# RalphAS/PeriodicSchurDecompositions.jl

Measured on NVIDIA B200. Metric: pschur!/sec batched (p=8,N=32); large-N FP64 % peak in large_n, higher is better.
Workload: dtype f64

## Files before the change

### periodicschurdecompositions.jl_b200/csrc/psd_capi.cu

```cuda
#include <algorithm>
#include <atomic>
#include <chrono>
#include <cstdio>
#include <cstdlib>
#include <cstring>
#include <mutex>
#include <string>
#include <thread>
#include <vector>

#include "../../include/psd_b200.h"
#include "psd_real_kernel.cuh"
#include "psd_checkpsd.cuh"
#include "psd_real_hess32.cuh"
#include "psd_cplx_qz.cuh"
#include "psd_rowhess.cuh"
#include "psd_dgemm.cuh"
#include "psd_large_hess.cuh"
#include "psd_ms.h"
#include "psd_rng.cuh"

namespace {

thread_local std::string g_err;
// ... 15 lines not shown
#define PSD_CUDA(call)                                                                     \
  do {                                                                                     \
    cudaError_t e__ = (call);                                                              \
    if (e__ != cudaSuccess)                                                                \
      return fail(PSD_ERR_CUDA, std::string(#call) + ": " + cudaGetErrorString(e__));      \
  } while (0)

constexpr int kSlotsPerDevice = 3;

struct Slot {
  cudaStream_t stream = nullptr;
  double* dA = nullptr;
  double* dZ = nullptr;
  double* dEig = nullptr;
  int32_t* dInfo = nullptr;
  size_t capA = 0, capZ = 0, capEig = 0, capInfo = 0;
  double* hA = nullptr;
  double* hZ = nullptr;
  double* hEig = nullptr;
  int32_t* hInfo = nullptr;
  size_t hcapA = 0, hcapZ = 0, hcapEig = 0, hcapInfo = 0;
  unsigned long long* dCounter = nullptr;
  double* dScratch = nullptr;
  size_t capScratch = 0;
  double* dPacked = nullptr;
  size_t capPacked = 0;
  double* dPk[8] = {nullptr};
  size_t capPk[8] = {0};
  unsigned long long* dPhaseCtr = nullptr;
  void* dX[3] = {nullptr, nullptr, nullptr};
  size_t capX[3] = {0, 0, 0};
  void* hX[3] = {nullptr, nullptr, nullptr};
  size_t hcapX[3] = {0, 0, 0};
  unsigned char* dS = nullptr;
  size_t capS = 0;
  psd::ms::Workspace* ms = nullptr;
  int32_t* dIters = nullptr;
  int32_t* hIters = nullptr;
  size_t capIters = 0, hcapIters = 0;
  int32_t* curIters = nullptr;
  double* curTau = nullptr;
  long long* dProf = nullptr;
};

struct Device {
  int ordinal = 0;
  int sm_count = 0;
  Slot slots[kSlotsPerDevice];
  Slot user;
  cudaEvent_t userDone = nullptr;
};

}

struct KernelTimer {
  cudaEvent_t e0, e1;
  int kind;
  int ordinal;
};

struct psd_handle_s {
  std::vector<Device> devs;
  std::mutex mu;
  int64_t stats[8] = {0};
  bool profiling = false;
  std::vector<KernelTimer> timers;
  double gemm_flops = 0.0;
  double extra_launches = 0.0;
  psd::ms::Result ms_last;
  int32_t* iters_host = nullptr;
  std::mutex tmu;
};

namespace {

template <class T>
int ensure_dev(T*& ptr, size_t& cap, size_t bytes) {
  if (bytes <= cap) return PSD_OK;
  if (ptr) cudaFree(ptr);
  ptr = nullptr;
  cap = 0;
  PSD_CUDA(cudaMalloc((void**)&ptr, bytes));
  cap = bytes;
  return PSD_OK;
}
template <class T>
int ensure_pinned(T*& ptr, size_t& cap, size_t bytes) {
  if (bytes <= cap) return PSD_OK;
  if (ptr) cudaFreeHost(ptr);
  ptr = nullptr;
  cap = 0;
  PSD_CUDA(cudaHostAlloc((void**)&ptr, bytes, cudaHostAllocDefault));
  cap = bytes;
  return PSD_OK;
}

bool is_pinned(const void* p) {
  if (!p) return true;
  cudaPointerAttributes at;
  cudaError_t e = cudaPointerGetAttributes(&at, p);
  if (e != cudaSuccess) {
    cudaGetLastError();
    return false;
  }
  return at.type == cudaMemoryTypeHost || at.type == cudaMemoryTypeManaged;
}

struct ScopedKernelTimer {
  psd_handle_s* h;
  cudaStream_t st;
  KernelTimer t;
  bool on;
  ScopedKernelTimer(psd_handle_s* h_, const Device& dev, cudaStream_t st_, int kind) : h(h_), st(st_) {
    on = h->profiling;
    if (!on) return;
    t.kind = kind;
    t.ordinal = dev.ordinal;
    cudaEventCreate(&t.e0);
    cudaEventCreate(&t.e1);
    cudaEventRecord(t.e0, st);
  }
  ~ScopedKernelTimer() {
    if (!on) return;
    cudaEventRecord(t.e1, st);
    std::lock_guard<std::mutex> lk(h->tmu);
    h->timers.push_back(t);
  }
};

struct RealLaunchPlan {
  int use_smem = 0;
  int ldh = 0;
  int threads = 64;
  size_t smem_bytes = 0;
  int grid = 1;
  bool scratch = false;
};

int plan_real(const Device& dev, int n, int p, long long batch, bool wantZ, RealLaunchPlan& pl) {
  const long long small = psd::rp_small_doubles(n, p);
  const int ldh = (n % 2 == 0) ? n + 1 : n;
  const long long mats = (long long)p * ldh * n * (wantZ ? 2 : 1);
  const size_t need_smem = (size_t)(small + mats) * sizeof(double);
  cudaFuncAttributes fa;
  PSD_CUDA(cudaFuncGetAttributes(&fa, psd::rpschur_kernel));
  int optin = 0;
  PSD_CUDA(cudaDeviceGetAttribute(&optin, cudaDevAttrMaxSharedMemoryPerBlockOptin, dev.ordinal));
  const size_t max_dyn = (size_t)optin - fa.sharedSizeBytes;
  if (need_smem <= max_dyn) {
    pl.use_smem = 1;
    pl.ldh = ldh;
    pl.smem_bytes = need_smem;
    pl.scratch = false;
  } else {
    pl.use_smem = 0;
    pl.ldh = n;
    if ((size_t)small * sizeof(double) <= 96 * 1024) {
      pl.smem_bytes = (size_t)small * sizeof(double);
      pl.scratch = false;
    } else {
      pl.smem_bytes = 0;
      pl.scratch = true;
    }
  }
  int want = n * (wantZ ? 3 : 2);
  int threads = ((want + 31) / 32) * 32;
  threads = std::max(32, std::min(threads, 256));
  pl.threads = threads;
  PSD_CUDA(cudaFuncSetAttribute(psd::rpschur_kernel, cudaFuncAttributeMaxDynamicSharedMemorySize,
                                (int)max_dyn));
  int occ = 0;
  PSD_CUDA(cudaOccupancyMaxActiveBlocksPerMultiprocessor(&occ, psd::rpschur_kernel, threads,
                                                         pl.smem_bytes));
  if (occ < 1) return fail(PSD_ERR_UNSUPPORTED, "kernel does not fit on an SM");
  long long g = (long long)occ * dev.sm_count;
  pl.grid = (int)std::max(1LL, std::min(g, batch));
  return PSD_OK;
}

struct RealCall {
  int n, p, left, wantT, wantZ, maxitfac, reduce_only, skip_reduce;
  int z_preset = 0;
};

constexpr int kLargeN = 192;

constexpr long long kEigChunk = 65536;

int launch_real_eig32(psd_handle_s* h, Device& dev, Slot& aux, cudaStream_t stream, const RealCall& rc,
                      long long batch, double* dA, double* dEig, int32_t* dInfo) {
  const int n = rc.n, p = rc.p;
  const size_t nn = (size_t)n * n;
  const size_t psize = (size_t)psd::pk_problem_size(n, p);
  long long chunk_max = kEigChunk;
  if (const char* ev = dbg_env("PSD_EIG_CHUNK")) chunk_max = std::max(1LL, atoll(ev));
  const long long chunk = std::min(batch, chunk_max);
  int e = ensure_dev(aux.dPacked, aux.capPacked, (size_t)chunk * psd::pk_problem_stride(n, p) * sizeof(double));
  if (e) return e;
  if (!aux.dCounter) PSD_CUDA(cudaMalloc((void**)&aux.dCounter, 2 * sizeof(unsigned long long)));
  if (!aux.dPhaseCtr) PSD_CUDA(cudaMalloc((void**)&aux.dPhaseCtr, 16 * sizeof(unsigned long long)));
  int optin = 0;
  PSD_CUDA(cudaDeviceGetAttribute(&optin, cudaDevAttrMaxSharedMemoryPerBlockOptin, dev.ordinal));
  struct Phase {
    int n, stop, wpb, grid;
    size_t smem;
    void (*kern)(psd::EigParams);
  };
  std::vector<Phase> phases;
  {
    std::vector<int> orders{n};
    if (n >= 24 && !dbg_env("PSD_NO_PHASES"))
      for (int k = 1; k <= 5; k++) orders.push_back(n - k * (n / 8));
    bool special = (n == 32 && p == 8 && !dbg_env("PSD_NO_SPECIAL"));
    if (const char* ev = dbg_env("PSD_PHASES")) {
      orders.assign(1, n);
      for (const char* c = ev; *c;) {
        int v = atoi(c);
        if (v > 1 && v < orders.back()) orders.push_back(v);
        while (*c && *c != ',') c++;
        if (*c == ',') c++;
      }
    }
    for (size_t k = 0; k < orders.size(); k++) {
      Phase ph;
      ph.n = orders[k];
      ph.stop = (k + 1 < orders.size()) ? orders[k + 1] : 0;
      ph.kern = psd::rpqr_eig32_kernel_t<0, 0>;
      if (special && k == 0) ph.kern = psd::rpqr_eig32_kernel_t<32, 8>;
      int wmax = 8;
      if (k > 0) {
        const char* lr = dbg_env("PSD_LOWREG");
        const int mode = lr ? atoi(lr) : 168;
        if (mode == 168) { ph.kern = psd::rpqr_eig32_kernel_r168; wmax = 3; }
        if (mode == 128) { ph.kern = psd::rpqr_eig32_kernel_r128; wmax = 4; }
      }
      cudaFuncAttributes fa;
      PSD_CUDA(cudaFuncGetAttributes(&fa, ph.kern));
      const size_t max_dyn = (size_t)optin - fa.sharedSizeBytes;
      const size_t pbytes = (size_t)psd::pk_problem_size(ph.n, p) * sizeof(double);
      PSD_CUDA(cudaFuncSetAttribute(ph.kern, cudaFuncAttributeMaxDynamicSharedMemorySize, (int)max_dyn));
      PSD_CUDA(cudaFuncSetAttribute(ph.kern, cudaFuncAttributePreferredSharedMemoryCarveout,
                                    (int)cudaSharedmemCarveoutMaxShared));
      int best_w = 0, best_total = 0;
      for (int w = 1; w <= wmax; w++) {
        if ((size_t)w * pbytes > max_dyn) break;
        int occ = 0;
        PSD_CUDA(cudaOccupancyMaxActiveBlocksPerMultiprocessor(&occ, ph.kern, w * 32, (size_t)w * pbytes));
        if (dbg_env("PSD_GEN_PROF")) fprintf(stderr, "[psd eig32 occ] order %d w %d -> %d CTAs/SM\n", ph.n, w, occ);
        if (occ * w > best_total || (occ * w == best_total && w > best_w)) {
          best_total = occ * w;
          best_w = w;
        }
      }
      if (best_w < 1) return fail(PSD_ERR_UNSUPPORTED, "packed problem does not fit in shared memory");
      if (const char* ev = dbg_env("PSD_PHASE_WPB")) {
        const int w = atoi(ev);
        if (k > 0 && w >= 1 && (size_t)w * pbytes <= max_dyn) {
          best_w = w;
          best_total = w * 4;
        }
      }
      ph.wpb = best_w;
      ph.smem = (size_t)best_w * pbytes;
      ph.grid = (best_total / best_w) * dev.sm_count;
      if (dbg_env("PSD_GEN_PROF"))
        fprintf(stderr, "[psd eig32 phase %zu] order %d stop %d: %d warps/CTA x %d CTAs/SM, %zu B smem/CTA, %d regs\n", k,
                ph.n, ph.stop, best_w, best_total / best_w, ph.smem, fa.numRegs);
      phases.push_back(ph);
    }
    if (phases.size() > 9) return fail(PSD_ERR_BAD_ARG, "too many phases");
    for (size_t k = 1; k < phases.size(); k++)
      if ((e = ensure_dev(aux.dPk[k - 1], aux.capPk[k - 1],
                          (size_t)chunk * psd::pk_problem_stride(phases[k].n, p) * sizeof(double))))
        return e;
  }
  for (long long off = 0; off < batch; off += chunk) {
    const long long nb = std::min(chunk, batch - off);
    PSD_CUDA(cudaMemsetAsync(aux.dCounter, 0, 2 * sizeof(unsigned long long), stream));
    if (rc.skip_reduce) {
      RealLaunchPlan pl;
      e = plan_real(dev, n, p, nb, false, pl);
      if (e) return e;
      if (!pl.use_smem) return fail(PSD_ERR_UNSUPPORTED, "eig32 path expects shared-memory staging");
      psd::RpschurParams P;
      P.n = n; P.p = p; P.batch = nb;
      P.left = rc.left; P.wantT = 0; P.wantZ = 0; P.maxitfac = 30;
      P.A = dA + (size_t)off * p * nn; P.Z = nullptr; P.eig = nullptr; P.info = nullptr; P.iters = nullptr;
      P.use_smem = pl.use_smem; P.ldh = pl.ldh;
      P.reduce_only = 1; P.skip_reduce = rc.skip_reduce; P.z_preset = 0;
      P.counter = aux.dCounter;
      P.scratch = nullptr; P.scratch_stride = 0;
      P.packed_out = aux.dPacked;
      P.tau = nullptr;
      ScopedKernelTimer tm(h, dev, stream, 0);
      psd::rpschur_kernel<<<pl.grid, pl.threads, pl.smem_bytes, stream>>>(P);
      PSD_CUDA(cudaGetLastError());
    } else {
      psd::Hess32Params R;
      R.n = n; R.p = p; R.batch = nb; R.left = rc.left;
      R.ld = (n % 2 == 0) ? n + 1 : n;
      R.A = dA + (size_t)off * p * nn;
      R.packed_out = aux.dPacked;
      R.counter = aux.dCounter;
      const bool pair = p >= 2 && !dbg_env("PSD_NO_HESS_PAIR");
      const bool special = n == 32 && p == 8 && !dbg_env("PSD_NO_SPECIAL");
      void (*hk)(psd::Hess32Params) =
          pair ? (special ? psd::rphess_pair32_kernel_t<32, 8> : psd::rphess_pair32_kernel_t<0, 0>)
               : (special ? psd::rphess_warp32_kernel_t<32, 8> : psd::rphess_warp32_kernel_t<0, 0>);
      const int wpp = pair ? 2 : 1;
      cudaFuncAttributes fh;
      PSD_CUDA(cudaFuncGetAttributes(&fh, hk));
      const size_t max_dyn1 = (size_t)optin - fh.sharedSizeBytes;
      const size_t per1 = (size_t)p * R.ld * n * sizeof(double);
      int wpb1 = (int)std::min<size_t>(8, max_dyn1 / per1);
      if (wpb1 < 1) return fail(PSD_ERR_UNSUPPORTED, "problem does not fit in shared memory");
      const size_t smem1 = (size_t)wpb1 * per1;
      PSD_CUDA(cudaFuncSetAttribute(hk, cudaFuncAttributeMaxDynamicSharedMemorySize,
                                    (int)max_dyn1));
      int occ1 = 0;
      PSD_CUDA(cudaOccupancyMaxActiveBlocksPerMultiprocessor(&occ1, hk, wpb1 * wpp * 32, smem1));
      if (occ1 < 1) return fail(PSD_ERR_UNSUPPORTED, "reduction kernel does not fit on an SM");
      const long long ctas1 = (nb + wpb1 - 1) / wpb1;
      const int grid1 = (int)std::max(1LL, std::min((long long)occ1 * dev.sm_count, ctas1));
      {
        ScopedKernelTimer tm(h, dev, stream, 0);
        hk<<<grid1, wpb1 * wpp * 32, smem1, stream>>>(R);
      }
      PSD_CUDA(cudaGetLastError());
    }
    PSD_CUDA(cudaMemsetAsync(aux.dPhaseCtr, 0, 16 * sizeof(unsigned long long), stream));
    {
      ScopedKernelTimer tm(h, dev, stream, 1);
      for (size_t k = 0; k < phases.size(); k++) {
        const Phase& ph = phases[k];
        psd::EigParams Q;
        Q.n = ph.n; Q.p = p; Q.batch = nb; Q.maxitfac = rc.maxitfac > 0 ? rc.maxitfac : 30;
        Q.packed = (k == 0) ? aux.dPacked : aux.dPk[k - 1];
        Q.packed_next = (k + 1 < phases.size()) ? aux.dPk[k] : nullptr;
        Q.n_full = n; Q.stop = ph.stop; Q.first_phase = (k == 0) ? 1 : 0;
        Q.eig = dEig + (size_t)off * 2 * n;
        Q.info = dInfo + off;
        Q.iters = aux.curIters ? aux.curIters + off : nullptr;
        Q.counter = aux.dPhaseCtr + k;
        Q.force_safe = dbg_env("PSD_EIG32_SAFE") ? 1 : 0;
        const long long ctas = (nb + ph.wpb - 1) / ph.wpb;
        const int grid2 = (int)std::max(1LL, std::min((long long)ph.grid, ctas));
        ph.kern<<<grid2, ph.wpb * 32, ph.smem, stream>>>(Q);
      }
    }
    PSD_CUDA(cudaGetLastError());
    {
      std::lock_guard<std::mutex> lk(h->tmu);
      h->extra_launches += (double)(phases.size() - 1);
    }
    __atomic_fetch_add(&h->stats[0], (int64_t)2, __ATOMIC_RELAXED);
  }
  __atomic_fetch_add(&h->stats[1], (int64_t)batch, __ATOMIC_RELAXED);
  return PSD_OK;
}


int launch_real_large(psd_handle_s* h, Device& dev, Slot& aux, cudaStream_t stream, const RealCall& rc,
                      long long batch, double* dA, double* dZ, double* dEig, int32_t* dInfo);
bool large_feasible(const Device& dev, int n, int p);

int launch_real(psd_handle_s* h, Device& dev, Slot& aux, cudaStream_t stream, const RealCall& rc,
                long long batch, double* dA, double* dZ, double* dEig, int32_t* dInfo) {
  if (batch == 0) return PSD_OK;
  RealLaunchPlan pl;
  const bool wantZ = rc.wantZ && dZ;
  if (rc.n >= kLargeN && !rc.skip_reduce && !aux.curTau && !dbg_env("PSD_DISABLE_LARGE") && large_feasible(dev, rc.n, rc.p))
    return launch_real_large(h, dev, aux, stream, rc, batch, dA, dZ, dEig, dInfo);
  if (!rc.wantT && !wantZ && !rc.reduce_only && rc.n <= 32 && rc.p >= 3 && !dbg_env("PSD_DISABLE_EIG32"))
    return launch_real_eig32(h, dev, aux, stream, rc, batch, dA, dEig, dInfo);
  int e = plan_real(dev, rc.n, rc.p, batch, wantZ, pl);
  if (e) return e;
  if (!aux.dCounter) PSD_CUDA(cudaMalloc((void**)&aux.dCounter, 2 * sizeof(unsigned long long)));
  PSD_CUDA(cudaMemsetAsync(aux.dCounter, 0, sizeof(unsigned long long), stream));
  psd::RpschurParams P;
  P.n = rc.n; P.p = rc.p; P.batch = batch;
  P.left = rc.left; P.wantT = rc.wantT; P.wantZ = wantZ ? 1 : 0;
  P.maxitfac = rc.maxitfac > 0 ? rc.maxitfac : 30;
  P.A = dA; P.Z = wantZ ? dZ : nullptr; P.eig = dEig; P.info = dInfo; P.iters = aux.curIters;
  P.use_smem = pl.use_smem; P.ldh = pl.ldh;
  P.reduce_only = rc.reduce_only; P.skip_reduce = rc.skip_reduce; P.z_preset = rc.z_preset;
  P.counter = aux.dCounter;
  P.scratch = nullptr; P.scratch_stride = 0;
  P.packed_out = nullptr;
  P.tau = aux.curTau;
  if (pl.scratch) {
    size_t stride = (size_t)psd::rp_small_doubles(rc.n, rc.p);
    e = ensure_dev(aux.dScratch, aux.capScratch, stride * sizeof(double) * pl.grid);
    if (e) return e;
    P.scratch = aux.dScratch;
    P.scratch_stride = (long long)stride;
  }
  {
    ScopedKernelTimer tm(h, dev, stream, 1);
    psd::rpschur_kernel<<<pl.grid, pl.threads, pl.smem_bytes, stream>>>(P);
  }
  PSD_CUDA(cudaGetLastError());
  __atomic_fetch_add(&h->stats[0], (int64_t)1, __ATOMIC_RELAXED);
  __atomic_fetch_add(&h->stats[pl.use_smem ? 1 : 2], (int64_t)batch, __ATOMIC_RELAXED);
  return PSD_OK;
}


bool large_feasible(const Device& dev, int n, int p) {
  if (p > psd::LH_MAXP) return false;
  const int nb = psd::lh_panel_width(p);
  int R = (n + dev.sm_count - 1) / dev.sm_count;
  R = (R + 3) & ~3;
  if (R > psd::LH_RMAX) return false;
  int optin = 0;
  if (cudaDeviceGetAttribute(&optin, cudaDevAttrMaxSharedMemoryPerBlockOptin, dev.ordinal) != cudaSuccess) return false;
  const size_t smem = ((size_t)p * nb * nb + n) * sizeof(double);
  cudaFuncAttributes fa;
  if (cudaFuncGetAttributes(&fa, psd::rphess_panel_kernel) != cudaSuccess) return false;
  if (smem + fa.sharedSizeBytes > (size_t)optin) return false;
  if (cudaFuncSetAttribute(psd::rphess_panel_kernel, cudaFuncAttributeMaxDynamicSharedMemorySize, (int)smem) != cudaSuccess) {
    cudaGetLastError();
    return false;
  }
  int occ = 0;
  if (cudaOccupancyMaxActiveBlocksPerMultiprocessor(&occ, psd::rphess_panel_kernel, psd::LH_THREADS, smem) != cudaSuccess || occ < 1) {
    cudaGetLastError();
    return false;
  }
  return true;
}

int launch_team_iteration(psd_handle_s* h, Device& dev, Slot& aux, cudaStream_t stream, const RealCall& rc,
                          long long batch, double* dA, double* dZ, double* dEig, int32_t* dInfo) {
  const int n = rc.n, p = rc.p;
  const bool wantZ = rc.wantZ && dZ;
  int e;
  const size_t cnt = (size_t)batch * n;
  if ((e = ensure_dev(aux.dX[0], aux.capX[0], cnt * 16))) return e;
  if ((e = ensure_dev(aux.dX[1], aux.capX[1], cnt * 8))) return e;
  if ((e = ensure_dev(aux.dX[2], aux.capX[2], cnt * 8))) return e;
  psd::GpqzParams<double> P;
  P.n = n; P.p = p; P.batch = batch; P.left = rc.left; P.wantT = rc.wantT; P.wantZ = wantZ ? 1 : 0;
  P.maxitfac = 4 * (rc.maxitfac > 0 ? rc.maxitfac : 30);
  P.skip_reduce = 1; P.reduce_only = 0;
  P.S = nullptr;
  P.A = dA; P.Z = wantZ ? dZ : nullptr;
  P.alpha = (psd::cplx*)aux.dX[0]; P.beta = (double*)aux.dX[1]; P.scale = (long long*)aux.dX[2];
  P.info = dInfo;
  P.use_smem = 0; P.ldh = n; P.debug = 0; P.counter = nullptr; P.blocked_stage1 = 0; P.windowed_stage2 = 0; P.windowed_qz = 0;
  P.deep = 4;
  if (const char* ev = dbg_env("PSD_DEEP_U")) P.deep = atoi(ev);
  auto kern = psd::gpschur_team_kernel<double>;
  size_t smem = (size_t)((psd::cq_small_doubles(n, p) + 1) & ~1LL) * sizeof(double);
  if (!dbg_env("PSD_NO_WINDOWED_QZ")) {
    P.windowed_qz = 1;
    smem += (size_t)psd::qzw_work_doubles(p, psd::S3_K_TEAM) * sizeof(double);
  }
  PSD_CUDA(cudaFuncSetAttribute(kern, cudaFuncAttributeMaxDynamicSharedMemorySize, (int)smem));
  int occ = 0;
  PSD_CUDA(cudaOccupancyMaxActiveBlocksPerMultiprocessor(&occ, kern, 256, smem));
  if (occ < 1) return fail(PSD_ERR_UNSUPPORTED, "team kernel does not fit on an SM");
  int zp = 1;
  void* args[] = {&P, &zp};
  int ctas = dev.sm_count;
  if (const char* ev = dbg_env("PSD_TEAM_CTAS")) ctas = std::max(1, std::min(atoi(ev), dev.sm_count * occ));
  {
    ScopedKernelTimer tm(h, dev, stream, 1);
    PSD_CUDA(cudaLaunchCooperativeKernel((void*)kern, dim3(ctas), dim3(256), args, smem, stream));
  }
  psd::gvalues_kernel<<<std::min<long long>(1024, (long long)(cnt + 255) / 256), 256, 0, stream>>>(
      (const psd::cplx*)aux.dX[0], (const double*)aux.dX[1], (const long long*)aux.dX[2], dEig, (long long)cnt);
  PSD_CUDA(cudaGetLastError());
  __atomic_fetch_add(&h->stats[0], (int64_t)2, __ATOMIC_RELAXED);
  return PSD_OK;
}

int launch_real_large(psd_handle_s* h, Device& dev, Slot& aux, cudaStream_t stream, const RealCall& rc,
                      long long batch, double* dA, double* dZ, double* dEig, int32_t* dInfo) {
  const int n = rc.n, p = rc.p;
  const size_t nn = (size_t)n * n;
  const bool wantZ = rc.wantZ && dZ;
  int e = ensure_dev(aux.dScratch, aux.capScratch,
                     (psd::lh_work_doubles(n, p) + (size_t)psd::rp_small_doubles(n, p) * 2) * sizeof(double));
  if (e) return e;
  double* work = aux.dScratch + (size_t)psd::rp_small_doubles(n, p) * 2;
  if (!aux.ms) aux.ms = psd::ms::ws_create();
  const bool scaled = p <= psd::ms::kMaxPeriod && !dbg_env("PSD_NO_PRESCALE");
  const bool use_ms = psd::ms::supported(n, p) && !rc.reduce_only && !dbg_env("PSD_DISABLE_MS");
  bool team_needed = false;
  for (long long b = 0; b < batch; b++) {
    double* Ab = dA + (size_t)b * p * nn;
    double* Zb = wantZ ? dZ + (size_t)b * p * nn : nullptr;
    double* Ap[psd::LH_MAXP];
    double* Qp[psd::LH_MAXP];
    for (int j = 1; j <= p; j++) {
      Ap[j - 1] = Ab + (size_t)((rc.left ? (p + 1 - j) : j) - 1) * nn;
      const int s = (rc.left && j > 1) ? (p + 2 - j) : j;
      Qp[j - 1] = Zb ? Zb + (size_t)(s - 1) * nn : nullptr;
    }
    if (scaled) PSD_CUDA(psd::ms::prescale(stream, aux.ms, n, p, Ap));
    double fl = 0.0;
    std::vector<ScopedKernelTimer*> open(4, nullptr);
    auto mark = [&](int kind, int phase) {
      if (phase == 0) {
        open[kind] = new ScopedKernelTimer(h, dev, stream, kind);
      } else {
        delete open[kind];
        open[kind] = nullptr;
      }
    };
    long long* dprof = nullptr;
    if (dbg_env("PSD_PANEL_PROF")) {
      if (!aux.dProf) PSD_CUDA(cudaMalloc((void**)&aux.dProf, 8 * sizeof(long long)));
      PSD_CUDA(cudaMemsetAsync(aux.dProf, 0, 8 * sizeof(long long), stream));
      dprof = aux.dProf;
    }
    cudaError_t ce = psd::rphess_large(stream, dev.sm_count, n, p, Ap, Zb ? Qp : nullptr, work, &fl, mark, dprof);
    if (dprof) {
      long long hp[8];
      PSD_CUDA(cudaMemcpyAsync(hp, dprof, sizeof(hp), cudaMemcpyDeviceToHost, stream));
      PSD_CUDA(cudaStreamSynchronize(stream));
      fprintf(stderr, "[psd panel cycles, CTA 0] s1+s2 %lld | wait S2 %lld | s3 %lld | wait S3 %lld | s4 head+gemv %lld | s4 tail %lld\n",
              hp[0], hp[1], hp[2], hp[3], hp[4], hp[5]);
    }
    for (auto* t : open) delete t;
    if (ce != cudaSuccess) return fail(PSD_ERR_CUDA, std::string("large-N reduction: ") + cudaGetErrorString(ce));
    {
      std::lock_guard<std::mutex> lk(h->tmu);
      h->gemm_flops += fl;
    }
    __atomic_fetch_add(&h->stats[0], (int64_t)((n + 63) / 64) * (1 + 7 * p), __ATOMIC_RELAXED);
    if (rc.reduce_only) {
      if (scaled) PSD_CUDA(psd::ms::postscale(stream, aux.ms, n, p, Ap, 1, nullptr));
      continue;
    }
    if (use_ms) {
      PSD_CUDA(cudaMemsetAsync(dInfo + b, 0, sizeof(int32_t), stream));
      psd::ms::Result res;
      {
        ScopedKernelTimer tm(h, dev, stream, 1);
        ce = psd::ms::iterate(stream, dev.sm_count, aux.ms, n, p, Ap, Zb ? Qp : nullptr, rc.wantT, wantZ ? 1 : 0,
                              rc.maxitfac, dEig + (size_t)b * 2 * n, dInfo + b, h->profiling ? 1 : 0, &res);
      }
      if (ce != cudaSuccess) return fail(PSD_ERR_CUDA, std::string("large-N iteration: ") + cudaGetErrorString(ce));
      {
        std::lock_guard<std::mutex> lk(h->tmu);
        h->ms_last = res;
      }
      __atomic_fetch_add(&h->stats[0], (int64_t)res.launches, __ATOMIC_RELAXED);
      if (res.status == 0) {
        if (scaled) PSD_CUDA(psd::ms::postscale(stream, aux.ms, n, p, Ap, rc.wantT, dEig + (size_t)b * 2 * n));
        continue;
      }
    }
    if (batch == 1) {
      team_needed = true;
    } else {
      RealCall r1 = rc;
      if ((e = launch_team_iteration(h, dev, aux, stream, r1, 1, Ab, Zb, dEig + (size_t)b * 2 * n, dInfo + b))) return e;
      if (scaled) PSD_CUDA(psd::ms::postscale(stream, aux.ms, n, p, Ap, rc.wantT, dEig + (size_t)b * 2 * n));
    }
  }
  if (team_needed) {
    if ((e = launch_team_iteration(h, dev, aux, stream, rc, 1, dA, dZ, dEig, dInfo))) return e;
    if (scaled) {
      double* Ap[psd::LH_MAXP];
      for (int j = 1; j <= p; j++) Ap[j - 1] = dA + (size_t)((rc.left ? (p + 1 - j) : j) - 1) * nn;
      PSD_CUDA(psd::ms::postscale(stream, aux.ms, n, p, Ap, rc.wantT, dEig));
    }
  }
  __atomic_fetch_add(&h->stats[2], (int64_t)batch, __ATOMIC_RELAXED);
  return PSD_OK;
}

int drain_slots(Device& dev, int code) {
  const std::string keep = g_err;
  for (int k = 0; k < kSlotsPerDevice; k++)
    if (dev.slots[k].stream) cudaStreamSynchronize(dev.slots[k].stream);
  cudaGetLastError();
  g_err = keep;
  return code;
}
#define PSD_SHARD_CUDA(call)                                                                        \
  do {                                                                                              \
    cudaError_t e__ = (call);                                                                       \
    if (e__ != cudaSuccess)                                                                         \
      return drain_slots(dev, fail(PSD_ERR_CUDA, std::string(#call) + ": " + cudaGetErrorString(e__))); \
  } while (0)

int run_real_shard(psd_handle_s* h, Device& dev, const RealCall& rc, long long first, long long count,
                   double* A, double* Z, double* eig, int32_t* info, bool pinned,
                   int64_t* bytes_h2d, int64_t* bytes_d2h) {
  if (count <= 0) return PSD_OK;
  PSD_SHARD_CUDA(cudaSetDevice(dev.ordinal));
  const size_t nn = (size_t)rc.n * rc.n;
  const size_t per = nn * rc.p;
  const bool wantZ = rc.wantZ && Z;
  const bool outT = rc.wantT || rc.reduce_only;
  long long chunk = std::max<long long>(1, (2048LL << 20) / (long long)(per * sizeof(double)));
  if (!pinned) chunk = std::max<long long>(1, std::min<long long>(chunk, (512LL << 20) / (long long)(per * sizeof(double))));
  chunk = std::min(chunk, count);
  if (!pinned && (size_t)count * per * sizeof(double) >= (64u << 20) && count >= 8)
    chunk = std::min(chunk, (count + 3) / 4);
  int si = 0;
  int rcode = PSD_OK;
  struct Pending {
    bool any = false;
    double *dstA = nullptr, *dstZ = nullptr, *dstEig = nullptr;
    int32_t *dstInfo = nullptr, *dstIters = nullptr;
    size_t bytesA = 0, bytesEig = 0, bytesInfo = 0, bytesIters = 0;
  } pend[kSlotsPerDevice];
  auto flush = [&](int k) {
    Pending& q = pend[k];
    if (!q.any) return;
    Slot& s = dev.slots[k];
    if (q.dstA) std::memcpy(q.dstA, s.hA, q.bytesA);
    if (q.dstZ) std::memcpy(q.dstZ, s.hZ, q.bytesA);
    if (q.dstEig) std::memcpy(q.dstEig, s.hEig, q.bytesEig);
    if (q.dstInfo) std::memcpy(q.dstInfo, s.hInfo, q.bytesInfo);
    if (q.dstIters) std::memcpy(q.dstIters, s.hIters, q.bytesIters);
    q = Pending();
  };
  long long nb = 0, next = (count > chunk) ? std::max<long long>(1, chunk / (pinned ? 16 : 2)) : chunk;
  for (long long off = 0; off < count && rcode == PSD_OK; off += nb, si = (si + 1) % kSlotsPerDevice) {
    nb = std::min(next, count - off);
    next = std::min(chunk, next * 4);
// ... 885 lines not shown
```

### periodicschurdecompositions.jl_b200/csrc/psd_real_hess32.cuh

```cuda
#pragma once
#include "psd_real_eig32.cuh"

namespace psd {

struct Hess32Params {
  int n, p;
  long long batch;
  int left;
  int ld;
  const double* A;
  double* packed_out;
  unsigned long long* counter;
};

PSD_DEV void hess32_step(double* Aj, double* Am, int n, int ld, int r0, int col, int lane) {
  double* xc = Aj + col * ld;
  const double alpha = xc[r0];
  const double xr = (lane > r0 && lane < n) ? xc[lane] : 0.0;
  double ssq = warp_sum(xr * xr);
  if (ssq == 0.0) {
    const double amax = warp_max(fabs(xr));
    if (amax == 0.0) return;
  }
  double nn = fma(alpha, alpha, ssq);
// ... 33 lines not shown
    const double sl = g * (dl0 + dl1), sr = g * (dr0 + dr1);
    if (la) cl[r0] = fma(sl, u0, cl[r0]);
    if (rw) ar[r0 * ld] = fma(sr, u0, ar[r0 * ld]);
#pragma unroll 2
    for (int k = r0 + 1; k < n; k += 2) {
      const bool p1 = k + 1 < n;
      const double x0 = xc[k], x1 = p1 ? xc[k + 1] : 0.0;
      const double l0 = cl[k], l1 = p1 ? cl[k + 1] : 0.0;
      const double q0 = ar[k * ld], q1 = p1 ? ar[(k + 1) * ld] : 0.0;
      if (la) {
        cl[k] = fma(sl, x0, l0);
        if (p1) cl[k + 1] = fma(sl, x1, l1);
      }
      if (rw) {
        ar[k * ld] = fma(sr, x0, q0);
        if (p1) ar[(k + 1) * ld] = fma(sr, x1, q1);
      }
    }
    __syncwarp();
    if (lane == r0) xc[lane] = beta;
    else if (lane > r0 && lane < n) xc[lane] = 0.0;
    __syncwarp();
    return;
  }
  if (lane > col && lane < n) {
    double* a = Aj + lane * ld;
    double d0 = u0 * a[r0], d1 = 0.0, d2 = 0.0, d3 = 0.0;
#pragma unroll 2
    for (int k = r0 + 1; k < n; k += 4) {
      const bool p1 = k + 1 < n, p2 = k + 2 < n, p3 = k + 3 < n;
      const double x0 = xc[k], x1 = p1 ? xc[k + 1] : 0.0, x2 = p2 ? xc[k + 2] : 0.0, x3 = p3 ? xc[k + 3] : 0.0;
      const double a0 = a[k], a1 = p1 ? a[k + 1] : 0.0, a2 = p2 ? a[k + 2] : 0.0, a3 = p3 ? a[k + 3] : 0.0;
      d0 = fma(x0, a0, d0); d1 = fma(x1, a1, d1); d2 = fma(x2, a2, d2); d3 = fma(x3, a3, d3);
    }
    const double s = g * ((d0 + d1) + (d2 + d3));
    a[r0] = fma(s, u0, a[r0]);
#pragma unroll 2
    for (int k = r0 + 1; k < n; k += 4) {
      const bool p1 = k + 1 < n, p2 = k + 2 < n, p3 = k + 3 < n;
      const double x0 = xc[k], x1 = p1 ? xc[k + 1] : 0.0, x2 = p2 ? xc[k + 2] : 0.0, x3 = p3 ? xc[k + 3] : 0.0;
      const double a0 = a[k], a1 = p1 ? a[k + 1] : 0.0, a2 = p2 ? a[k + 2] : 0.0, a3 = p3 ? a[k + 3] : 0.0;
      a[k] = fma(s, x0, a0);
      if (p1) a[k + 1] = fma(s, x1, a1);
      if (p2) a[k + 2] = fma(s, x2, a2);
      if (p3) a[k + 3] = fma(s, x3, a3);
    }
  }
  if (Am == Aj) __syncwarp();
  if (lane < n) {
    double* a = Am + lane;
    double d0 = a[r0 * ld] * u0, d1 = 0.0, d2 = 0.0, d3 = 0.0;
#pragma unroll 2
    for (int k = r0 + 1; k < n; k += 4) {
      const bool p1 = k + 1 < n, p2 = k + 2 < n, p3 = k + 3 < n;
      const double x0 = xc[k], x1 = p1 ? xc[k + 1] : 0.0, x2 = p2 ? xc[k + 2] : 0.0, x3 = p3 ? xc[k + 3] : 0.0;
      const double a0 = a[k * ld], a1 = p1 ? a[(k + 1) * ld] : 0.0, a2 = p2 ? a[(k + 2) * ld] : 0.0,
                   a3 = p3 ? a[(k + 3) * ld] : 0.0;
      d0 = fma(a0, x0, d0); d1 = fma(a1, x1, d1); d2 = fma(a2, x2, d2); d3 = fma(a3, x3, d3);
    }
    const double s = g * ((d0 + d1) + (d2 + d3));
    a[r0 * ld] = fma(s, u0, a[r0 * ld]);
#pragma unroll 2
    for (int k = r0 + 1; k < n; k += 4) {
      const bool p1 = k + 1 < n, p2 = k + 2 < n, p3 = k + 3 < n;
      const double x0 = xc[k], x1 = p1 ? xc[k + 1] : 0.0, x2 = p2 ? xc[k + 2] : 0.0, x3 = p3 ? xc[k + 3] : 0.0;
      const double a0 = a[k * ld], a1 = p1 ? a[(k + 1) * ld] : 0.0, a2 = p2 ? a[(k + 2) * ld] : 0.0,
                   a3 = p3 ? a[(k + 3) * ld] : 0.0;
      a[k * ld] = fma(s, x0, a0);
      if (p1) a[(k + 1) * ld] = fma(s, x1, a1);
      if (p2) a[(k + 2) * ld] = fma(s, x2, a2);
      if (p3) a[(k + 3) * ld] = fma(s, x3, a3);
    }
  }
  __syncwarp();
  if (lane == r0) xc[lane] = beta;
  else if (lane > r0 && lane < n) xc[lane] = 0.0;
  __syncwarp();
}

extern __shared__ __align__(16) double psd_smem_hess[];

template <int NN, int PP>
__global__ void __launch_bounds__(256) rphess_warp32_kernel_t(Hess32Params P) {
  const int lane = threadIdx.x & 31, warp = threadIdx.x >> 5;
  const int n = NN ? NN : P.n, p = PP ? PP : P.p, ld = NN ? (NN % 2 == 0 ? NN + 1 : NN) : P.ld;
  const size_t nn = (size_t)n * n;
  const int fs = ld * n;
  double* S = psd_smem_hess + (size_t)warp * p * fs;
  const int psize = pk_problem_size(n, p);
  for (;;) {
    long long b = 0;
    if (lane == 0) b = (long long)atomicAdd(P.counter, 1ULL);
    b = __shfl_sync(0xffffffffu, b, 0);
    if (b >= P.batch) break;
    const double* Ab = P.A + (size_t)b * p * nn;
    for (int j = 0; j < p; j++) {
      const double* src = Ab + (size_t)(P.left ? (p - 1 - j) : j) * nn;
      double* dst = S + j * fs;
      if (lane < n)
        for (int c = 0; c < n; c++) {
          const unsigned sa = (unsigned)__cvta_generic_to_shared(dst + c * ld + lane);
          asm volatile("cp.async.ca.shared.global [%0], [%1], 8;" ::"r"(sa), "l"(src + c * n + lane));
        }
    }
    asm volatile("cp.async.wait_all;" ::: "memory");
    __syncwarp();
    int escale = 0;
    for (int j = 0; j < p; j++) {
      double* dst = S + j * fs;
      double m = 0.0;
      if (lane < n)
        for (int c = 0; c < n; c++) m = fmax(m, fabs(dst[c * ld + lane]));
      m = warp_max(m);
      if (m > 0.0 && m < 1.7e308) {
        int e;
        (void)frexp(m, &e);
        if (e != 0) {
          const double sc = scalbn(1.0, (-e > 1000) ? 1000 : -e);
          if (lane < n)
            for (int c = 0; c < n; c++) dst[c * ld + lane] *= sc;
          escale += e;
        }
      }
    }
    __syncwarp();
    for (int i = 0; i < n - 1; i++) {
      for (int j = p - 1; j >= 1; j--) hess32_step(S + j * fs, S + (j - 1) * fs, n, ld, i, i, lane);
      if (n - (i + 1) > 1) hess32_step(S, S + (p - 1) * fs, n, ld, i + 1, i, lane);
    }
    double* dstb = P.packed_out + (size_t)b * (psize + PK_STATE);
    if (lane == 0) dstb[psize] = (double)escale;
    for (int j = 0; j < p; j++) {
      const int kl = (j == 0) ? 3 : 1;
      const int keep = (j == 0) ? 1 : 0;
      double* dst = dstb + ((j == 0) ? 0 : pk_size(3, n) + (j - 1) * pk_size(1, n));
      const double* src = S + j * fs;
      for (int c = 0; c < n; c++) {
        const int off = pk_off(kl, c);
        if (lane <= c + kl && lane < n) dst[off + lane] = (lane <= c + keep) ? src[c * ld + lane] : 0.0;
      }
    }
    __syncwarp();
  }
}

PSD_DEV void pair_barrier(int id) { asm volatile("bar.sync %0, 64;" ::"r"(id) : "memory"); }

PSD_DEV void hess32_step_pair(double* Aj, double* Am, int n, int ld, int r0, int col, int lane, int role, int barid) {
  double* xc = Aj + col * ld;
  const double alpha = xc[r0];
  const double xr = (lane > r0 && lane < n) ? xc[lane] : 0.0;
  double ssq = warp_sum(xr * xr);
  if (ssq == 0.0) {
    const double amax = warp_max(fabs(xr));
    if (amax == 0.0) return;
  }
  double nn = fma(alpha, alpha, ssq);
  double sc = 1.0;
  if (!(ssq > 1e-280 && nn < 1e280)) {
    const double m = fmax(warp_max(fabs(xr)), fabs(alpha));
    sc = pow2_rescale(m);
    const double y = xr * sc;
    ssq = warp_sum(y * y);
    nn = fma(alpha * sc, alpha * sc, ssq);
  }
  const double al = alpha * sc;
  const double nrm = nn * fast_rsqrt(nn);
  const double betas = -copysign(nrm, al);
  const double u0s = al - betas;
  const double gs = -2.0 * fast_rcp(fma(u0s, u0s, ssq));
  double g = gs, u0 = u0s, beta = betas;
  if (sc != 1.0) {
    g = gs * sc * sc;
    u0 = u0s / sc;
    beta = betas / sc;
  }
  if (role == 0) {
    if (lane > col && lane < n) {
      double* a = Aj + lane * ld;
      double d0 = u0 * a[r0], d1 = 0.0, d2 = 0.0, d3 = 0.0;
#pragma unroll 2
      for (int k = r0 + 1; k < n; k += 4) {
        const bool p1 = k + 1 < n, p2 = k + 2 < n, p3 = k + 3 < n;
        const double x0 = xc[k], x1 = p1 ? xc[k + 1] : 0.0, x2 = p2 ? xc[k + 2] : 0.0, x3 = p3 ? xc[k + 3] : 0.0;
        const double a0 = a[k], a1 = p1 ? a[k + 1] : 0.0, a2 = p2 ? a[k + 2] : 0.0, a3 = p3 ? a[k + 3] : 0.0;
        d0 = fma(x0, a0, d0); d1 = fma(x1, a1, d1); d2 = fma(x2, a2, d2); d3 = fma(x3, a3, d3);
      }
      const double s = g * ((d0 + d1) + (d2 + d3));
      a[r0] = fma(s, u0, a[r0]);
#pragma unroll 2
      for (int k = r0 + 1; k < n; k += 4) {
        const bool p1 = k + 1 < n, p2 = k + 2 < n, p3 = k + 3 < n;
        const double x0 = xc[k], x1 = p1 ? xc[k + 1] : 0.0, x2 = p2 ? xc[k + 2] : 0.0, x3 = p3 ? xc[k + 3] : 0.0;
        const double a0 = a[k], a1 = p1 ? a[k + 1] : 0.0, a2 = p2 ? a[k + 2] : 0.0, a3 = p3 ? a[k + 3] : 0.0;
        a[k] = fma(s, x0, a0);
        if (p1) a[k + 1] = fma(s, x1, a1);
        if (p2) a[k + 2] = fma(s, x2, a2);
        if (p3) a[k + 3] = fma(s, x3, a3);
      }
    }
  } else {
    if (lane < n) {
      double* a = Am + lane;
      double d0 = a[r0 * ld] * u0, d1 = 0.0, d2 = 0.0, d3 = 0.0;
#pragma unroll 2
      for (int k = r0 + 1; k < n; k += 4) {
        const bool p1 = k + 1 < n, p2 = k + 2 < n, p3 = k + 3 < n;
        const double x0 = xc[k], x1 = p1 ? xc[k + 1] : 0.0, x2 = p2 ? xc[k + 2] : 0.0, x3 = p3 ? xc[k + 3] : 0.0;
        const double a0 = a[k * ld], a1 = p1 ? a[(k + 1) * ld] : 0.0, a2 = p2 ? a[(k + 2) * ld] : 0.0,
                     a3 = p3 ? a[(k + 3) * ld] : 0.0;
        d0 = fma(a0, x0, d0); d1 = fma(a1, x1, d1); d2 = fma(a2, x2, d2); d3 = fma(a3, x3, d3);
      }
      const double s = g * ((d0 + d1) + (d2 + d3));
      a[r0 * ld] = fma(s, u0, a[r0 * ld]);
#pragma unroll 2
      for (int k = r0 + 1; k < n; k += 4) {
        const bool p1 = k + 1 < n, p2 = k + 2 < n, p3 = k + 3 < n;
        const double x0 = xc[k], x1 = p1 ? xc[k + 1] : 0.0, x2 = p2 ? xc[k + 2] : 0.0, x3 = p3 ? xc[k + 3] : 0.0;
        const double a0 = a[k * ld], a1 = p1 ? a[(k + 1) * ld] : 0.0, a2 = p2 ? a[(k + 2) * ld] : 0.0,
                     a3 = p3 ? a[(k + 3) * ld] : 0.0;
        a[k * ld] = fma(s, x0, a0);
        if (p1) a[(k + 1) * ld] = fma(s, x1, a1);
        if (p2) a[(k + 2) * ld] = fma(s, x2, a2);
        if (p3) a[(k + 3) * ld] = fma(s, x3, a3);
      }
    }
  }
  pair_barrier(barid);
  if (role == 0) {
    if (lane == r0) xc[lane] = beta;
    else if (lane > r0 && lane < n) xc[lane] = 0.0;
  }
}

template <int NN, int PP>
__global__ void __launch_bounds__(512) rphess_pair32_kernel_t(Hess32Params P) {
  const int lane = threadIdx.x & 31, warp = threadIdx.x >> 5;
  const int grp = warp >> 1, role = warp & 1, barid = 1 + grp;
  const int n = NN ? NN : P.n, p = PP ? PP : P.p, ld = NN ? (NN % 2 == 0 ? NN + 1 : NN) : P.ld;
  const size_t nn = (size_t)n * n;
  const int fs = ld * n;
  double* S = psd_smem_hess + (size_t)grp * p * fs;
  __shared__ long long s_b[8];
  __shared__ int s_e[8];
  const int psize = pk_problem_size(n, p);
  for (;;) {
    if (role == 0 && lane == 0) s_b[grp] = (long long)atomicAdd(P.counter, 1ULL);
    pair_barrier(barid);
    const long long b = s_b[grp];
    if (b >= P.batch) break;
    const double* Ab = P.A + (size_t)b * p * nn;
    int escale = 0;
    for (int j = role; j < p; j += 2) {
      const double* src = Ab + (size_t)(P.left ? (p - 1 - j) : j) * nn;
      double* dst = S + j * fs;
      if (lane < n)
        for (int c = 0; c < n; c++) {
          const unsigned sa = (unsigned)__cvta_generic_to_shared(dst + c * ld + lane);
          asm volatile("cp.async.ca.shared.global [%0], [%1], 8;" ::"r"(sa), "l"(src + c * n + lane));
        }
    }
    asm volatile("cp.async.wait_all;" ::: "memory");
    __syncwarp();
    for (int j = role; j < p; j += 2) {
      double* dst = S + j * fs;
      double m = 0.0;
      if (lane < n)
        for (int c = 0; c < n; c++) m = fmax(m, fabs(dst[c * ld + lane]));
      m = warp_max(m);
      if (m > 0.0 && m < 1.7e308) {
        int e;
        (void)frexp(m, &e);
        if (e != 0) {
          const double sc = scalbn(1.0, (-e > 1000) ? 1000 : -e);
          if (lane < n)
            for (int c = 0; c < n; c++) dst[c * ld + lane] *= sc;
          escale += e;
        }
      }
    }
    if (role == 1 && lane == 0) s_e[grp] = escale;
    pair_barrier(barid);
    if (role == 0) escale += s_e[grp];
    for (int i = 0; i < n - 1; i++) {
      for (int j = p - 1; j >= 1; j--) hess32_step_pair(S + j * fs, S + (j - 1) * fs, n, ld, i, i, lane, role, barid);
      if (n - (i + 1) > 1) hess32_step_pair(S, S + (p - 1) * fs, n, ld, i + 1, i, lane, role, barid);
    }
    pair_barrier(barid);
    double* dstb = P.packed_out + (size_t)b * (psize + PK_STATE);
    if (role == 0 && lane == 0) dstb[psize] = (double)escale;
    for (int j = role; j < p; j += 2) {
      const int kl = (j == 0) ? 3 : 1;
      const int keep = (j == 0) ? 1 : 0;
      double* dst = dstb + ((j == 0) ? 0 : pk_size(3, n) + (j - 1) * pk_size(1, n));
      const double* src = S + j * fs;
      for (int c = 0; c < n; c++) {
        const int off = pk_off(kl, c);
        if (lane <= c + kl && lane < n) dst[off + lane] = (lane <= c + keep) ? src[c * ld + lane] : 0.0;
      }
    }
  }
}

}
```

Measured before the change: 246,100.

## Add three-warp look-ahead Hessenberg reduction kernel pipelined with mbarrier ring

```diff
diff --git a/periodicschurdecompositions.jl_b200/csrc/psd_capi.cu b/periodicschurdecompositions.jl_b200/csrc/psd_capi.cu
--- a/periodicschurdecompositions.jl_b200/csrc/psd_capi.cu
+++ b/periodicschurdecompositions.jl_b200/csrc/psd_capi.cu
@@ -341,26 +341,50 @@
       R.A = dA + (size_t)off * p * nn;
       R.packed_out = aux.dPacked;
       R.counter = aux.dCounter;
-      const bool pair = p >= 2 && !dbg_env("PSD_NO_HESS_PAIR");
       const bool special = n == 32 && p == 8 && !dbg_env("PSD_NO_SPECIAL");
-      void (*hk)(psd::Hess32Params) =
-          pair ? (special ? psd::rphess_pair32_kernel_t<32, 8> : psd::rphess_pair32_kernel_t<0, 0>)
-               : (special ? psd::rphess_warp32_kernel_t<32, 8> : psd::rphess_warp32_kernel_t<0, 0>);
-      const int wpp = pair ? 2 : 1;
-      cudaFuncAttributes fh;
-      PSD_CUDA(cudaFuncGetAttributes(&fh, hk));
-      const size_t max_dyn1 = (size_t)optin - fh.sharedSizeBytes;
-      const size_t per1 = (size_t)p * R.ld * n * sizeof(double);
-      int wpb1 = (int)std::min<size_t>(8, max_dyn1 / per1);
-      if (wpb1 < 1) return fail(PSD_ERR_UNSUPPORTED, "problem does not fit in shared memory");
-      const size_t smem1 = (size_t)wpb1 * per1;
-      PSD_CUDA(cudaFuncSetAttribute(hk, cudaFuncAttributeMaxDynamicSharedMemorySize,
-                                    (int)max_dyn1));
-      int occ1 = 0;
-      PSD_CUDA(cudaOccupancyMaxActiveBlocksPerMultiprocessor(&occ1, hk, wpb1 * wpp * 32, smem1));
-      if (occ1 < 1) return fail(PSD_ERR_UNSUPPORTED, "reduction kernel does not fit on an SM");
+      struct Shape {
+        void (*k)(psd::Hess32Params);
+        int wpp, wpb, occ;
+        size_t smem;
+      };
+      const size_t staged = (size_t)p * R.ld * n * sizeof(double);
+      auto shape = [&](void (*k)(psd::Hess32Params), int wpp, size_t per, Shape& sh) -> int {
+        cudaFuncAttributes fh;
+        PSD_CUDA(cudaFuncGetAttributes(&fh, k));
+        const size_t max_dyn = (size_t)optin - fh.sharedSizeBytes;
+        sh.k = k;
+        sh.wpp = wpp;
+        sh.wpb = (int)std::min<size_t>(std::min(8, fh.maxThreadsPerBlock / (32 * wpp)), max_dyn / per);
+        sh.occ = 0;
+        if (sh.wpb < 1) return PSD_OK;
+        sh.smem = (size_t)sh.wpb * per;
+        PSD_CUDA(cudaFuncSetAttribute(k, cudaFuncAttributeMaxDynamicSharedMemorySize, (int)max_dyn));
+        PSD_CUDA(cudaOccupancyMaxActiveBlocksPerMultiprocessor(&sh.occ, k, sh.wpb * wpp * 32, sh.smem));
+        return PSD_OK;
+      };
+      Shape hs;
+      if (p == 1) {
+        if ((e = shape(special ? psd::rphess_warp32_kernel_t<32, 8> : psd::rphess_warp32_kernel_t<0, 0>, 1, staged, hs)))
+          return e;
+      } else {
+        if ((e = shape(psd::rphess_pair32_kernel_t<0, 0>, 2, staged, hs))) return e;
+        if (p >= 7) {
+          Shape as;
+          if ((e = shape(special ? psd::rphess_ahead32_kernel_t<32, 8> : psd::rphess_ahead32_kernel_t<0, 0>,
+                         psd::AHEAD_WARPS, psd::ahead_problem_doubles(n, p, R.ld) * sizeof(double), as)))
+            return e;
+          if (as.occ > 0 && as.wpb * as.occ >= hs.wpb * hs.occ) hs = as;
+        }
+      }
+      if (hs.occ < 1) return fail(PSD_ERR_UNSUPPORTED, "reduction kernel does not fit on an SM");
+      const int wpb1 = hs.wpb, wpp = hs.wpp, occ1 = hs.occ;
+      const size_t smem1 = hs.smem;
+      void (*hk)(psd::Hess32Params) = hs.k;
       const long long ctas1 = (nb + wpb1 - 1) / wpb1;
       const int grid1 = (int)std::max(1LL, std::min((long long)occ1 * dev.sm_count, ctas1));
+      if (dbg_env("PSD_GEN_PROF"))
+        fprintf(stderr, "[psd hess32] %d warps/problem, %d problems/CTA x %d CTAs/SM, %zu B smem/CTA\n", wpp, wpb1,
+                occ1, smem1);
       {
         ScopedKernelTimer tm(h, dev, stream, 0);
         hk<<<grid1, wpb1 * wpp * 32, smem1, stream>>>(R);
diff --git a/periodicschurdecompositions.jl_b200/csrc/psd_real_hess32.cuh b/periodicschurdecompositions.jl_b200/csrc/psd_real_hess32.cuh
--- a/periodicschurdecompositions.jl_b200/csrc/psd_real_hess32.cuh
+++ b/periodicschurdecompositions.jl_b200/csrc/psd_real_hess32.cuh
@@ -359,4 +359,307 @@
   }
 }
 
-}
+constexpr int AHEAD_RING = 8;
+constexpr int AHEAD_ENT = 68;
+constexpr int AHEAD_CTL = 28;
+constexpr int AHEAD_WARPS = 3;
+
+__host__ __device__ inline size_t ahead_problem_doubles(int n, int p, int ld) {
+  return (size_t)p * ld * n + AHEAD_RING * AHEAD_ENT + AHEAD_CTL;
+}
+
+PSD_DEV unsigned ahead_u32(const void* q) { return (unsigned)__cvta_generic_to_shared(q); }
+PSD_DEV void ahead_mbar_init(unsigned long long* b, int cnt) {
+  asm volatile("mbarrier.init.shared::cta.b64 [%0], %1;" ::"r"(ahead_u32(b)), "r"(cnt) : "memory");
+}
+PSD_DEV void ahead_mbar_arrive(unsigned long long* b) {
+  asm volatile("mbarrier.arrive.shared::cta.b64 _, [%0];" ::"r"(ahead_u32(b)) : "memory");
+}
+PSD_DEV void ahead_mbar_wait(unsigned long long* b, unsigned parity) {
+  unsigned ok;
+  do {
+    asm volatile(
+        "{\n.reg .pred q;\nmbarrier.try_wait.parity.shared::cta.b64 q, [%1], %2;\nselp.u32 %0, 1, 0, q;\n}\n"
+        : "=r"(ok)
+        : "r"(ahead_u32(b)), "r"(parity)
+        : "memory");
+  } while (!ok);
+}
+PSD_DEV void group_barrier(int id, int nthr) { asm volatile("bar.sync %0, %1;" ::"r"(id), "r"(nthr) : "memory"); }
+
+struct AheadPos {
+  int slot = 0;
+  unsigned phase = 0;
+  bool used = false;
+  PSD_DEV void advance(int slots) {
+    if (++slot == slots) {
+      slot = 0;
+      phase ^= 1u;
+      used = true;
+    }
+  }
+};
+
+PSD_DEV double ahead_tail_dot(const double* a, int st, const double* xc, int r0, int len, double d0, double (&v)[32],
+                              double (&x)[32]) {
+#pragma unroll
+  for (int t = 0; t < 32; t++) {
+    const bool in = t < len;
+    const int k = in ? r0 + 1 + t : r0;
+    x[t] = in ? xc[k] : 0.0;
+    v[t] = in ? a[k * st] : 0.0;
+  }
+  double d1 = 0.0, d2 = 0.0, d3 = 0.0;
+#pragma unroll
+  for (int c = 0; c < 8; c++) {
+    if (4 * c < len) {
+      d0 = fma(x[4 * c], v[4 * c], d0);
+      d1 = fma(x[4 * c + 1], v[4 * c + 1], d1);
+      d2 = fma(x[4 * c + 2], v[4 * c + 2], d2);
+      d3 = fma(x[4 * c + 3], v[4 * c + 3], d3);
+    }
+  }
+  return (d0 + d1) + (d2 + d3);
+}
+
+PSD_DEV void ahead_chain_step(double* Aj, double* Am, int n, int ld, int r0, int col, int lane, double* ring,
+                              unsigned long long* full, unsigned long long* empty, const AheadPos& q) {
+  double* ent = ring + q.slot * AHEAD_ENT;
+  if (q.used) ahead_mbar_wait(empty + q.slot, q.phase ^ 1u);
+  double* xc = Aj + col * ld;
+  const double alpha = xc[r0];
+  const double xr = (lane > r0 && lane < n) ? xc[lane] : 0.0;
+  double ssq = warp_sum(xr * xr);
+  if (ssq == 0.0) {
+    const double amax = warp_max(fabs(xr));
+    if (amax == 0.0) {
+      if (lane == 0) {
+        ent[66] = 1.0;
+        ahead_mbar_arrive(full + q.slot);
+      }
+      return;
+    }
+  }
+  double nn = fma(alpha, alpha, ssq);
+  double sc = 1.0;
+  if (!(ssq > 1e-280 && nn < 1e280)) {
+    const double m = fmax(warp_max(fabs(xr)), fabs(alpha));
+    sc = pow2_rescale(m);
+    const double y = xr * sc;
+    ssq = warp_sum(y * y);
+    nn = fma(alpha * sc, alpha * sc, ssq);
+  }
+  const double al = alpha * sc;
+  const double nrm = nn * fast_rsqrt(nn);
+  const double betas = -copysign(nrm, al);
+  const double u0s = al - betas;
+  const double gs = -2.0 * fast_rcp(fma(u0s, u0s, ssq));
+  double g = gs, u0 = u0s, beta = betas;
+  if (sc != 1.0) {
+    g = gs * sc * sc;
+    u0 = u0s / sc;
+    beta = betas / sc;
+  }
+  if (lane < n) {
+    double* a = Am + lane;
+    double v[32], x[32];
+    const double ar0 = a[r0 * ld];
+    const double s = g * ahead_tail_dot(a, ld, xc, r0, n - r0 - 1, ar0 * u0, v, x);
+    a[r0 * ld] = fma(s, u0, ar0);
+    ent[32 + lane] = s;
+  }
+  if (lane > r0 && lane < n) ent[lane] = xr;
+  if (lane == 0) {
+    ent[64] = u0;
+    ent[65] = g;
+    ent[66] = 0.0;
+  }
+  __threadfence_block();
+  __syncwarp();
+  if (lane == 0) ahead_mbar_arrive(full + q.slot);
+  if (lane == r0) xc[lane] = beta;
+  else if (lane > r0 && lane < n) xc[lane] = 0.0;
+  __syncwarp();
+}
+
+PSD_DEV void ahead_left_step(double* Aj, int n, int r0, int col, int ld, int lane, const double* ring,
+                             unsigned long long* full, unsigned long long* empty, unsigned long long* mid,
+                             const AheadPos& q, const AheadPos& prev, bool first) {
+  if (!first) {
+    ahead_mbar_wait(mid + prev.slot, prev.phase);
+    if (lane == 0) ahead_mbar_arrive(empty + prev.slot);
+  }
+  const double* ent = ring + q.slot * AHEAD_ENT;
+  ahead_mbar_wait(full + q.slot, q.phase);
+  if (ent[66] != 0.0) return;
+  const double u0 = ent[64], g = ent[65];
+  const double* xc = ent;
+  if (lane > col && lane < n) {
+    double* a = Aj + lane * ld;
+    const int len = n - r0 - 1;
+    double v[32], x[32];
+    const double ar0 = a[r0];
+    const double s = g * ahead_tail_dot(a, 1, xc, r0, len, u0 * ar0, v, x);
+    a[r0] = fma(s, u0, ar0);
+#pragma unroll
+    for (int t = 0; t < 31; t++)
+      if (t < len) a[r0 + 1 + t] = fma(s, x[t], v[t]);
+  }
+  __threadfence_block();
+  __syncwarp();
+}
+
+PSD_DEV void ahead_right_step(double* Am, int n, int r0, int ld, int lane, const double* ring,
+                              unsigned long long* full, unsigned long long* empty, unsigned long long* mid,
+                              const AheadPos& q) {
+  const double* ent = ring + q.slot * AHEAD_ENT;
+  ahead_mbar_wait(full + q.slot, q.phase);
+  if (ent[66] == 0.0 && lane < n) {
+    const double s = ent[32 + lane];
+    const double* xc = ent;
+    double* a = Am + lane;
+    const int len = n - r0 - 1;
+    double v[32], x[32];
+#pragma unroll
+    for (int t = 0; t < 31; t++) {
+      const bool in = t < len;
+      const int k = in ? r0 + 1 + t : r0;
+      x[t] = in ? xc[k] : 0.0;
+      v[t] = in ? a[k * ld] : 0.0;
+    }
+#pragma unroll
+    for (int t = 0; t < 31; t++)
+      if (t < len) a[(r0 + 1 + t) * ld] = fma(s, x[t], v[t]);
+  }
+  __threadfence_block();
+  __syncwarp();
+  if (lane == 0) {
+    ahead_mbar_arrive(mid + q.slot);
+    ahead_mbar_arrive(empty + q.slot);
+  }
+}
+
+template <int NN, int PP>
+__global__ void __launch_bounds__(AHEAD_WARPS * 32 * 4) rphess_ahead32_kernel_t(Hess32Params P) {
+  const int lane = threadIdx.x & 31, warp = threadIdx.x >> 5;
+  constexpr int gw = AHEAD_WARPS;
+  const int grp = warp / gw, role = warp - grp * gw, barid = 1 + grp, nthr = gw * 32;
+  const int n = NN ? NN : P.n, p = PP ? PP : P.p, ld = NN ? (NN % 2 == 0 ? NN + 1 : NN) : P.ld;
+  const size_t nn = (size_t)n * n;
+  const int fs = ld * n;
+  double* S = psd_smem_hess + (size_t)grp * ahead_problem_doubles(n, p, ld);
+  double* ring = S + (size_t)p * fs;
+  unsigned long long* full = (unsigned long long*)(ring + AHEAD_RING * AHEAD_ENT);
+  unsigned long long* empty = full + AHEAD_RING;
+  unsigned long long* mid = empty + AHEAD_RING;
+  long long* s_b = (long long*)(mid + AHEAD_RING);
+  int* s_e = (int*)(s_b + 1);
+  const int slots = (p - 1 < AHEAD_RING) ? p - 1 : AHEAD_RING;
+  if (role == 0 && lane == 0)
+    for (int k = 0; k < slots; k++) {
+      ahead_mbar_init(full + k, 1);
+      ahead_mbar_init(empty + k, 2);
+      ahead_mbar_init(mid + k, 1);
+    }
+  __syncthreads();
+  const int psize = pk_problem_size(n, p);
+  AheadPos q;
+  for (;;) {
+    if (role == 0 && lane == 0) *s_b = (long long)atomicAdd(P.counter, 1ULL);
+    group_barrier(barid, nthr);
+    const long long b = *s_b;
+    if (b >= P.batch) break;
+    const double* Ab = P.A + (size_t)b * p * nn;
+    int escale = 0;
+    for (int j = role; j < p; j += gw) {
+      const double* src = Ab + (size_t)(P.left ? (p - 1 - j) : j) * nn;
+      double* dst = S + j * fs;
+      if (lane < n)
+        for (int c = 0; c < n; c++) {
+          const unsigned sa = (unsigned)__cvta_generic_to_shared(dst + c * ld + lane);
+          asm volatile("cp.async.ca.shared.global [%0], [%1], 8;" ::"r"(sa), "l"(src + c * n + lane));
+        }
+    }
+    asm volatile("cp.async.wait_all;" ::: "memory");
+    __syncwarp();
+    for (int j = role; j < p; j += gw) {
+      double* dst = S + j * fs;
+      double m = 0.0;
+      if (lane < n)
+        for (int c = 0; c < n; c++) m = fmax(m, fabs(dst[c * ld + lane]));
+      m = warp_max(m);
+      if (m > 0.0 && m < 1.7e308) {
+        int e;
+        (void)frexp(m, &e);
+        if (e != 0) {
+          const double sc = scalbn(1.0, (-e > 1000) ? 1000 : -e);
+          if (lane < n)
+            for (int c = 0; c < n; c++) dst[c * ld + lane] *= sc;
+          escale += e;
+        }
+      }
+    }
+    if (lane == 0) s_e[role] = escale;
+    group_barrier(barid, nthr);
+    if (role == 0) {
+      for (int w = 1; w < gw; w++) escale += s_e[w];
+      for (int i = 0; i < n - 1; i++) {
+        for (int j = p - 1; j >= 1; j--) {
+          ahead_chain_step(S + j * fs, S + (j - 1) * fs, n, ld, i, i, lane, ring, full, empty, q);
+          q.advance(slots);
+        }
+        if (n - (i + 1) > 1) {
+          ahead_chain_step(S, S + (p - 1) * fs, n, ld, i + 1, i, lane, ring, full, empty, q);
+          q.advance(slots);
+        }
+      }
+    } else if (role == 1) {
+      AheadPos prev = q;
+      bool first = true;
+      for (int i = 0; i < n - 1; i++) {
+        for (int j = p - 1; j >= 1; j--) {
+          ahead_left_step(S + j * fs, n, i, i, ld, lane, ring, full, empty, mid, q, prev, first);
+          prev = q;
+          first = false;
+          q.advance(slots);
+        }
+        if (n - (i + 1) > 1) {
+          ahead_left_step(S, n, i + 1, i, ld, lane, ring, full, empty, mid, q, prev, first);
+          prev = q;
+          first = false;
+          q.advance(slots);
+        }
+      }
+      if (!first) {
+        ahead_mbar_wait(mid + prev.slot, prev.phase);
+        if (lane == 0) ahead_mbar_arrive(empty + prev.slot);
+      }
+    } else {
+      for (int i = 0; i < n - 1; i++) {
+        for (int j = p - 1; j >= 1; j--) {
+          ahead_right_step(S + (j - 1) * fs, n, i, ld, lane, ring, full, empty, mid, q);
+          q.advance(slots);
+        }
+        if (n - (i + 1) > 1) {
+          ahead_right_step(S + (p - 1) * fs, n, i + 1, ld, lane, ring, full, empty, mid, q);
+          q.advance(slots);
+        }
+      }
+    }
+    group_barrier(barid, nthr);
+    double* dstb = P.packed_out + (size_t)b * (psize + PK_STATE);
+    if (role == 0 && lane == 0) dstb[psize] = (double)escale;
+    for (int j = role; j < p; j += gw) {
+      const int kl = (j == 0) ? 3 : 1;
+      const int keep = (j == 0) ? 1 : 0;
+      double* dst = dstb + ((j == 0) ? 0 : pk_size(3, n) + (j - 1) * pk_size(1, n));
+      const double* src = S + j * fs;
+      for (int c = 0; c < n; c++) {
+        const int off = pk_off(kl, c);
+        if (lane <= c + kl && lane < n) dst[off + lane] = (lane <= c + keep) ? src[c * ld + lane] : 0.0;
+      }
+    }
+  }
+}
+
+}
```

Result: faster. 264,200 (median of 6 runs) (+7.4%).
